# TianxiangZhao/EdgeDisentangle_SSL

Measured on NVIDIA B200. Metric: DISGAT fwd+bwd edges/s, higher is better.
Workload: dtype f32

## Files before the change

### edgedisentangle_ssl_b200/_lib.py

```python
import ctypes
import os
from ctypes import POINTER, Structure, c_char_p, c_double, c_float, c_int, c_int32, c_int64, c_uint64, c_void_p

_PKG = os.path.dirname(os.path.abspath(__file__))
LIB_PATH = os.environ.get("EDIS_LIB") or os.path.join(_PKG, "libedis.so")


class EdisError(RuntimeError):
    pass


class LayerDesc(Structure):
    _fields_ = [("att", c_int32), ("C", c_int32), ("D", c_int32), ("Dv", c_int32),
                ("training", c_int32), ("p", c_float), ("seed", c_uint64), ("flags", c_int32),
                ("reserved", c_int32)]


ERR_STALE = -5
FLAG_PLAIN_MEAN = 1
FLAG_NO_GX = 2
FLAG_PHASE_DST, FLAG_PHASE_SRC, FLAG_PHASE_GX = 4, 8, 16


def _load():
    if not os.path.exists(LIB_PATH):
        raise ImportError(
            "libedis.so not found at %s: build it with `python -m edgedisentangle_ssl_b200.build` "
            "(nvcc, sm_100a).  This package has no CPU / PyTorch fallback." % LIB_PATH)
    return ctypes.CDLL(LIB_PATH)


lib = _load()

_i64p = POINTER(c_int64)
_i32p = POINTER(c_int32)
_f32p = POINTER(c_float)
_f64p = POINTER(c_double)
_descp = POINTER(LayerDesc)
_P = c_void_p

_BWD_ARGS = [c_void_p, _descp, _P, c_int64, _P, c_int64, _P, _P, c_int64, _P, _P, _P, _P, _P, _P, _P,
             _P, c_int64, _P, c_int64, _P, _P, c_int64, _P, _P, _P, c_int64, _P]

SIGNATURES = {
    "edis_last_error": (c_char_p, []),
    "edis_version": (c_char_p, []),
    "edis_build_adjacency_host": (c_int64, [c_int64, c_int64, _i64p, _i64p, _f64p, _i64p, _i64p, _f32p]),
    "edis_graph_create": (c_int, [c_int64, c_int64, _i64p, _i64p, c_int, c_int, POINTER(c_void_p)]),
    "edis_graph_create_rect": (c_int, [c_int64, c_int64, c_int64, _i64p, _i64p, c_int, c_int, POINTER(c_void_p)]),
    "edis_graph_destroy": (None, [c_void_p]),
    "edis_graph_info": (c_int, [c_void_p, _i64p]),
    "edis_graph_input_entries": (c_int64, [c_void_p]),
    "edis_graph_export": (c_int, [c_void_p, _i64p, _i32p, _i64p, _i64p, _i32p, _i32p]),
    "edis_graph_workspace_bytes": (c_int64, [c_void_p, c_int64]),
    "edis_edge_list_key": (c_uint64, [c_int64, c_int64, c_int64, _i64p, _i64p, c_int]),
    "edis_graph_save": (c_int, [c_void_p, c_char_p, c_uint64]),
    "edis_graph_load": (c_int, [c_char_p, c_uint64, c_int, c_int, c_int, POINTER(c_void_p)]),
    "edis_disga_fwd": (c_int, [c_void_p, _descp, _P, c_int64, _P, c_int64, _P, _P, c_int64, _P,
                               _P, _P, _P, _P, _P, _P, c_int64, _P]),
    "edis_disga_rec_bytes": (c_int64, [c_void_p, _descp]),
    "edis_disga_sign_bytes": (c_int64, [c_void_p, _descp]),
    "edis_disga_bwd": (c_int, _BWD_ARGS),
    "edis_disga_bwd_dst": (c_int, _BWD_ARGS),
    "edis_disga_bwd_src": (c_int, _BWD_ARGS),
    "edis_disga_sage_fwd": (c_int, [c_void_p, _descp, _P, c_int64, _P, c_int64, _P, _P, c_int64,
                                    _P, _P, _P, _P, _P, c_int64, _P]),
    "edis_disga_sage_bwd": (c_int, [c_void_p, _descp, _P, c_int64, _P, c_int64, _P, _P, c_int64,
                                    _P, _P, _P, _P, _P, _P, _P, c_int64, _P, c_int64, _P, _P, _P, _P, _P,
                                    c_int64, _P]),
    "edis_disga_sage_fused_gx": (c_int, [_descp]),
    "edis_pair_score_fwd": (c_int, [_descp, c_int64, c_int64, _P, _P, c_int32, c_int32, _P, c_int64,
                                    _P, c_int64, _P, _P, _P, _P]),
    "edis_pair_score_bwd": (c_int, [_descp, c_int64, c_int64, _P, _P, c_int32, c_int32, _P, c_int64,
                                    _P, c_int64, _P, _P, _P, _P, _P, _P, _P, _P]),
    "edis_pair_sign_bytes": (c_int64, [_descp, c_int64, c_int32, c_int32]),
    "edis_ssl_wmse_fwd": (c_int, [c_int64, c_int32, _P, _P, c_int64, c_int64, _P, _P, c_int64, _P]),
    "edis_ssl_wmse_bwd": (c_int, [c_int64, c_int32, _P, _P, c_int64, c_int64, _P, _P, _P]),
    "edis_nll_const_label_fwd": (c_int, [c_int64, c_int32, _P, c_int32, _P, _P, c_int64, _P]),
    "edis_nll_const_label_bwd": (c_int, [c_int64, c_int32, _P, c_int32, _P, _P, _P]),
    "edis_sp_softmax_fwd": (c_int, [c_int64, c_int64, _P, _P, _P, _P, _P, _P]),
    "edis_sp_softmax_bwd": (c_int, [c_int64, c_int64, _P, _P, _P, _P, _P, _P]),
    "edis_sp_matmul_fwd": (c_int, [c_int64, c_int64, c_int64, _P, _P, _P, _P, _P, _P]),
    "edis_sp_matmul_bwd": (c_int, [c_int64, c_int64, c_int64, _P, _P, _P, _P, _P, _P, _P, _P]),
    "edis_merge_pairs_host": (c_int64, [c_int64, _i64p, c_int64, _i64p, c_int64, _i64p, _i64p, _f32p]),
    "edis_rand_hits_host": (c_int64, [c_void_p, c_int64, c_int64, ctypes.c_uint32, _i64p, c_int64]),
}

for _name, (_res, _args) in SIGNATURES.items():
    _fn = getattr(lib, _name)
    _fn.restype = _res
    _fn.argtypes = _args


def last_error():
    return lib.edis_last_error().decode("utf-8", "replace")


def check(status, what):
    if status is not None and status < 0:
        raise EdisError("%s failed (%d): %s" % (what, status, last_error()))
    return status


def np_ptr(arr, ctype):
    return arr.ctypes.data_as(POINTER(ctype))


def version():
    return lib.edis_version().decode()
```

### edgedisentangle_ssl_b200/functional.py

```python
import ctypes

import torch

from . import _lib
from ._lib import LayerDesc, check, lib


def _stream():
    return ctypes.c_void_p(torch.cuda.current_stream().cuda_stream)


def _ptr(t):
    return ctypes.c_void_p(t.data_ptr()) if t is not None else None


def _off(t, col):
    return ctypes.c_void_p(t.data_ptr() + 4 * int(col))


def _rows(t, what):
    if t.dtype != torch.float32 or not t.is_cuda:
        raise _lib.EdisError("%s must be a float32 CUDA tensor (got %s on %s)" % (what, t.dtype, t.device))
    if t.dim() != 2 or t.stride(1) != 1:
        t = t.contiguous()
    return t, t.stride(0)


class KernelTimer:

    def __init__(self):
        self.enabled = False
        self.records = {}
        self.launches = 0

    def reset(self):
        self.records = {}
        self.launches = 0

    def durations_ms(self):
        return {k: [a.elapsed_time(b) for a, b, _ in v] for k, v in self.records.items()}

    def bytes(self):
        return {k: [m for _, _, m in v] for k, v in self.records.items()}


TIMER = KernelTimer()


def kernel_bytes(kind, n, nc, e, att, C, D, Fin=None, sage=False):
    CD = C * D
    score = 4 * C if att == 1 else 4 * CD
    agg_ref = 4 * Fin if sage else 4 * CD
    agg_own = 4 * CD if Fin is None else 4 * Fin
    wout = CD if Fin is None else C * Fin
    sign = CD // 8 if att == 3 else 0
    if kind == "fwd":
        alg = e * (score + agg_ref + 4 * C + 4) + 8 * CD * n
        moved = e * (score + agg_own + 4 * C + sign + 4) + n * (score + 4 * wout * (1 if Fin else 2) + 8 * C)
    elif kind == "bwd_dst":
        alg = e * (score + agg_ref + 4 * C + 4) + 8 * CD * n
        moved = (e * ((score if att == 2 else 0) + agg_own + 4 * C + 8 * C + sign + 4)
                 + n * (12 * wout + 2 * score + 8 * C))
    elif kind == "bwd_src":
        alg = e * (score + agg_ref) + 4 * CD * n
        moved = (e * ((score if att == 2 else 0) + 4 * wout + 8 * C + sign + 8)
                 + nc * (score + (4 * CD if Fin is None else 4 * Fin)))
    elif kind == "bwd_src_score":
        alg = e * score + 4 * CD * n
        moved = e * ((score if att == 2 else 0) + 8 * C + sign + 8) + nc * score
    else:
        alg = e * agg_ref
        moved = e * (4 * wout + 4 * C + 8) + nc * 4 * Fin
    return {"alg": int(alg), "moved": int(moved)}


class _timed:
    def __init__(self, name, graph, launches, nbytes=None):
        self.name, self.launches, self.nbytes = name, launches, nbytes

    def __enter__(self):
        if TIMER.enabled:
            self.start = torch.cuda.Event(enable_timing=True)
            self.end = torch.cuda.Event(enable_timing=True)
            self.start.record(torch.cuda.current_stream())
        return self

    def __exit__(self, *exc):
        if TIMER.enabled:
            self.end.record(torch.cuda.current_stream())
            TIMER.records.setdefault(self.name, []).append((self.start, self.end, self.nbytes))
            TIMER.launches += self.launches
        return False


def phase(name):
    return _timed("phase:" + name, None, 0, None)


def _desc(att, C, D, training=False, p=0.0, seed=0):
    return LayerDesc(att=att, C=C, D=D, Dv=D, training=1 if (training and p > 0) else 0, p=float(p),
                     seed=int(seed) & 0xFFFFFFFFFFFFFFFF)


def _edge_rec(graph, d, device):
    nbytes = check(lib.edis_disga_rec_bytes(graph.handle, ctypes.byref(d)), "edis_disga_rec_bytes")
    return torch.empty(int(nbytes), dtype=torch.uint8, device=device)


def _sign_rec(graph, d, device, wanted):
    if d.att != 3 or not wanted:
        return None
    nbytes = check(lib.edis_disga_sign_bytes(graph.handle, ctypes.byref(d)), "edis_disga_sign_bytes")
    return torch.empty(int(nbytes), dtype=torch.uint8, device=device)


def _workspace(graph, width, like):
    nbytes = graph.workspace_bytes(width)
    return torch.empty(nbytes, dtype=torch.uint8, device=like.device), nbytes


def disga_forward_raw(graph, d, P, ldp, Q, ldq, V, ldv, a, bias, device, want_sign):
    C, D = d.C, d.D
    CD = C * D
    n, e = graph.n, graph.e
    out = torch.empty(n, CD, dtype=torch.float32, device=device)
    hpre = torch.empty_like(out)
    edge_e = torch.empty(e, C, dtype=torch.float32, device=device)
    stats = torch.empty(n, 2 * C, dtype=torch.float32, device=device)
    ws, nbytes = _workspace(graph, CD + 2 * C, out)
    esign = _sign_rec(graph, d, device, want_sign)
    with _timed("disga_fwd", graph, 1 + (1 if graph.info["dst_slots"] else 0),
                kernel_bytes("fwd", n, graph.n_cols, e, d.att, C, D)):
        check(lib.edis_disga_fwd(graph.handle, ctypes.byref(d), P, ldp, Q, ldq, _ptr(a), V, ldv, _ptr(bias),
                                 _ptr(out), _ptr(hpre), _ptr(edge_e), _ptr(stats), _ptr(esign), _ptr(ws), nbytes,
                                 _stream()), "edis_disga_fwd")
    return out, hpre, edge_e, stats, esign


def disga_backward_raw(graph, d, P, ldp, Q, ldq, V, ldv, a, bias, hpre, edge_e, stats, esign, g_out, g_edge_e,
                       gP, ldgp, gQ, ldgq, ga, gV, ldgv, device):
    C, D, att = d.C, d.D, d.att
    CD = C * D
    n, e, nc = graph.n, graph.e, graph.n_cols
    edge_rec = _edge_rec(graph, d, device)
    gh = torch.empty(n, CD, dtype=torch.float32, device=device)
    ws, nbytes = _workspace(graph, 2 * CD + 2 * C, gh)
    args = (graph.handle, ctypes.byref(d), P, ldp, Q, ldq, _ptr(a), V, ldv, _ptr(bias),
            _ptr(hpre), _ptr(edge_e), _ptr(stats), _ptr(esign), _ptr(g_out), _ptr(g_edge_e), gP, ldgp, gQ, ldgq,
            _ptr(ga), gV, ldgv, _ptr(edge_rec), _ptr(gh), _ptr(ws), nbytes, _stream())
    with _timed("disga_bwd_dst", graph, 1 + (1 if graph.info["dst_slots"] else 0),
                kernel_bytes("bwd_dst", n, nc, e, att, C, D)):
        check(lib.edis_disga_bwd_dst(*args), "edis_disga_bwd_dst")
    with _timed("disga_bwd_src", graph, 1 + (2 if graph.info["src_slots"] else 0),
                kernel_bytes("bwd_src", n, nc, e, att, C, D)):
        check(lib.edis_disga_bwd_src(*args), "edis_disga_bwd_src")
    return gh


class DisGAFused(torch.autograd.Function):

    @staticmethod
    def forward(ctx, graph, att, C, D, proj, off_p, off_q, off_v, sdst, ssrc, a, bias, training, p, seed):
        proj, ld = _rows(proj, "proj")
        if att == 1:
            sdst, ssrc = sdst.contiguous(), ssrc.contiguous()
            P, Q, ldp, ldq = _ptr(sdst), _ptr(ssrc), C, C
        else:
            P, Q, ldp, ldq = _off(proj, off_p), _off(proj, off_q), ld, ld
        a = a.contiguous() if a is not None else None
        bias = bias.contiguous() if bias is not None else None
        if proj.shape[0] != graph.n_cols:
            raise _lib.EdisError("projection has %d rows, graph has %d source nodes" % (proj.shape[0], graph.n_cols))
        d = _desc(att, C, D, training, p, seed)
        out, hpre, edge_e, stats, esign = disga_forward_raw(graph, d, P, ldp, Q, ldq, _off(proj, off_v), ld, a, bias,
                                                            proj.device, any(ctx.needs_input_grad))
        ctx.graph, ctx.d, ctx.offs = graph, d, (off_p, off_q, off_v)
        ctx.has_a, ctx.has_bias = a is not None, bias is not None
        ctx.save_for_backward(proj, sdst, ssrc, a, bias, hpre, edge_e, stats, esign)
        ctx.set_materialize_grads(False)
        return out, edge_e

    @staticmethod
    def backward(ctx, g_out, g_edge_e):
        proj, sdst, ssrc, a, bias, hpre, edge_e, stats, esign = ctx.saved_tensors
        graph, d = ctx.graph, ctx.d
        C, D, att = d.C, d.D, d.att
        CD = C * D
        n, e, nc = graph.n, graph.e, graph.n_cols
        rect = nc > n
        off_p, off_q, off_v = ctx.offs
        ld, W, dev = proj.stride(0), proj.shape[1], proj.device
        if g_out is None:
            g_out = torch.zeros(n, CD, dtype=torch.float32, device=dev)
        g_out = g_out.contiguous()
        if g_edge_e is not None:
            g_edge_e = g_edge_e.contiguous()
        g_sd = g_ss = gq_sep = None
        if att == 1:
            g_proj = torch.zeros(nc, W, dtype=torch.float32, device=dev)
            g_sd = (torch.zeros if rect else torch.empty)(nc, C, dtype=torch.float32, device=dev)
            g_ss = torch.empty(nc, C, dtype=torch.float32, device=dev)
            P, Q, ldp, ldq = _ptr(sdst), _ptr(ssrc), C, C
            gP, gQ, ldgp, ldgq = _ptr(g_sd), _ptr(g_ss), C, C
        else:
            covered = CD * (3 if att == 3 else 2)
            g_proj = (torch.empty if W == covered and not rect else torch.zeros)(nc, W, dtype=torch.float32,
                                                                                 device=dev)
            P, Q, ldp, ldq = _off(proj, off_p), _off(proj, off_q), ld, ld
            gP, ldgp = _off(g_proj, off_p), W
            if off_q == off_p:
                gq_sep = torch.empty(nc, CD, dtype=torch.float32, device=dev)
                gQ, ldgq = _ptr(gq_sep), CD
            else:
                gQ, ldgq = _off(g_proj, off_q), W
        ga = torch.zeros(C, D, dtype=torch.float32, device=dev) if att == 3 else None
        gh = disga_backward_raw(graph, d, P, ldp, Q, ldq, _off(proj, off_v), ld, a, bias, hpre, edge_e, stats, esign,
                                g_out, g_edge_e, gP, ldgp, gQ, ldgq, ga, _off(g_proj, off_v), W, dev)
        if gq_sep is not None:
            g_proj[:, off_p:off_p + CD] += gq_sep
        gbias = gh.sum(0) if ctx.has_bias else None
        return (None, None, None, None, g_proj, None, None, None, g_sd, g_ss,
                ga if ctx.has_a else None, gbias, None, None, None)


def sage_forward_raw(graph, d, P, ldp, Q, ldq, X, a, want_sign):
    n, e, Fin, C = graph.n, graph.e, X.shape[1], d.C
    if X.shape[0] != graph.n_cols:
        raise _lib.EdisError("X has %d rows, graph has %d source nodes" % (X.shape[0], graph.n_cols))
    agg = torch.empty(n, C * Fin, dtype=torch.float32, device=X.device)
    edge_e = torch.empty(e, C, dtype=torch.float32, device=X.device)
    stats = torch.empty(n, 2 * C, dtype=torch.float32, device=X.device)
    ws, nbytes = _workspace(graph, C * Fin + 2 * C, X)
    esign = _sign_rec(graph, d, X.device, want_sign)
    plain = bool(d.flags & _lib.FLAG_PLAIN_MEAN)
    with _timed("disga_sage_fwd", graph, 1 + (1 if graph.info["dst_slots"] else 0),
                kernel_bytes("fwd", n, graph.n_cols, e, d.att, C, d.D, Fin, sage=not plain)):
        check(lib.edis_disga_sage_fwd(graph.handle, ctypes.byref(d), P, ldp, Q, ldq, _ptr(a), _ptr(X), X.stride(0),
                                      _ptr(agg), _ptr(edge_e), _ptr(stats), _ptr(esign), _ptr(ws), nbytes,
                                      _stream()),
              "edis_disga_sage_fwd")
    return agg, edge_e, stats, esign


def sage_backward_raw(graph, d, P, ldp, Q, ldq, X, a, agg, edge_e, stats, esign, g_agg, g_edge_e, gP, ldgp, gQ, ldgq,
                      ga, need_gx):
    C, D, att, Fin = d.C, d.D, d.att, d.Dv
    CD = C * D
    n, e, nc = graph.n, graph.e, graph.n_cols
    dev = X.device
    gX = torch.empty(nc, Fin, dtype=torch.float32, device=dev) if need_gx else None
    edge_rec = _edge_rec(graph, d, dev)
    gh = torch.empty(n, C * Fin, dtype=torch.float32, device=dev)
    ws, nbytes = _workspace(graph, 2 * CD + 2 * C + Fin, X)
    base = d.flags
    plain = bool(base & _lib.FLAG_PLAIN_MEAN)
    fused_gx = bool(lib.edis_disga_sage_fused_gx(ctypes.byref(d)))
    kb = lambda kind: kernel_bytes(kind, n, nc, e, att, C, D, Fin, sage=not plain)
    phases = [("disga_sage_bwd_dst", _lib.FLAG_PHASE_DST, 1 + (1 if graph.info["dst_slots"] else 0), kb("bwd_dst")),
              ("disga_sage_bwd_src", _lib.FLAG_PHASE_SRC, 1 + (1 if graph.info["src_slots"] else 0),
               kb("bwd_src" if (fused_gx and need_gx) else "bwd_src_score"))]
    if need_gx and not fused_gx:
        phases.append(("disga_sage_bwd_gx", _lib.FLAG_PHASE_GX, 1 + (1 if graph.info["src_slots"] else 0),
                       kb("bwd_gx")))
    for name, bit, nl, nb in phases:
        d.flags = base | bit
        with _timed(name, graph, nl, nb):
            check(lib.edis_disga_sage_bwd(graph.handle, ctypes.byref(d), P, ldp, Q, ldq, _ptr(a), _ptr(X),
                                          X.stride(0), _ptr(agg), _ptr(edge_e), _ptr(stats), _ptr(esign), _ptr(g_agg),
                                          _ptr(g_edge_e), gP, ldgp, gQ, ldgq, _ptr(ga), _ptr(gX),
                                          _ptr(edge_rec), _ptr(gh), _ptr(ws), nbytes, _stream()),
                  "edis_disga_sage_bwd")
    d.flags = base
    return gX


class SageFused(torch.autograd.Function):

    @staticmethod
    def forward(ctx, graph, att, C, D, proj, off_p, off_q, sdst, ssrc, a, X, training, p, seed, plain):
        X, ldx = _rows(X, "X")
        if att == 1:
            sdst, ssrc = sdst.contiguous(), ssrc.contiguous()
            P, Q, ldp, ldq = _ptr(sdst), _ptr(ssrc), C, C
        else:
            proj, ld = _rows(proj, "proj")
            P, Q, ldp, ldq = _off(proj, off_p), _off(proj, off_q), ld, ld
        a = a.contiguous() if a is not None else None
        d = _desc(att, C, D, training, p, seed)
        d.Dv = X.shape[1]
        d.flags = (_lib.FLAG_PLAIN_MEAN if plain else 0) | (0 if ctx.needs_input_grad[10] else _lib.FLAG_NO_GX)
        agg, edge_e, stats, esign = sage_forward_raw(graph, d, P, ldp, Q, ldq, X, a, any(ctx.needs_input_grad))
        ctx.graph, ctx.d, ctx.offs, ctx.plain = graph, d, (off_p, off_q), bool(plain)
        ctx.has_a = a is not None
        ctx.save_for_backward(proj, sdst, ssrc, a, X, agg, edge_e, stats, esign)
        ctx.set_materialize_grads(False)
        return agg, edge_e

    @staticmethod
    def backward(ctx, g_agg, g_edge_e):
        proj, sdst, ssrc, a, X, agg, edge_e, stats, esign = ctx.saved_tensors
        graph, d = ctx.graph, ctx.d
        C, D, att = d.C, d.D, d.att
        CD = C * D
        n, nc = graph.n, graph.n_cols
        rect = nc > n
        off_p, off_q = ctx.offs
        dev = X.device
        if g_agg is None:
            g_agg = torch.zeros_like(agg)
        g_agg = g_agg.contiguous()
        if g_edge_e is not None:
            g_edge_e = g_edge_e.contiguous()
        g_proj = g_sd = g_ss = gq_sep = None
        if att == 1:
            g_sd = (torch.zeros if rect else torch.empty)(nc, C, dtype=torch.float32, device=dev)
            g_ss = torch.empty(nc, C, dtype=torch.float32, device=dev)
            P, Q, ldp, ldq = _ptr(sdst), _ptr(ssrc), C, C
            gP, gQ, ldgp, ldgq = _ptr(g_sd), _ptr(g_ss), C, C
        else:
            ld, W = proj.stride(0), proj.shape[1]
            covered = CD * (2 if att == 3 else 1)
            g_proj = (torch.empty if W == covered and not rect else torch.zeros)(nc, W, dtype=torch.float32,
                                                                                 device=dev)
            P, Q, ldp, ldq = _off(proj, off_p), _off(proj, off_q), ld, ld
            gP, ldgp = _off(g_proj, off_p), W
            if off_q == off_p:
                gq_sep = torch.empty(nc, CD, dtype=torch.float32, device=dev)
                gQ, ldgq = _ptr(gq_sep), CD
            else:
                gQ, ldgq = _off(g_proj, off_q), W
        need_gx = not (d.flags & _lib.FLAG_NO_GX)
        ga = torch.zeros(C, D, dtype=torch.float32, device=dev) if att == 3 else None
        gX = sage_backward_raw(graph, d, P, ldp, Q, ldq, X, a, agg, edge_e, stats, esign, g_agg, g_edge_e, gP, ldgp,
                               gQ, ldgq, ga, need_gx)
        if gq_sep is not None:
            g_proj[:, off_p:off_p + CD] += gq_sep
        return (None, None, None, None, g_proj, None, None, g_sd, g_ss, ga if ctx.has_a else None, gX,
                None, None, None, None)


PROJ3X_MIN_ROWS = 65536


def use_proj3x(n_rows):
    import os
    mode = os.environ.get("EDIS_PROJ3X", "auto")
    return mode == "1" or (mode != "0" and n_rows >= PROJ3X_MIN_ROWS)


def _tf32_hi(t):
    return ((t.view(torch.int32) + 0x1000) & -0x2000).view(torch.float32)


def _xt_g(x, g, chunks=256):
    n = x.shape[0]
    if n < chunks * 1024:
        return x.t() @ g
    m = (n // chunks) * chunks
    out = torch.bmm(x[:m].view(chunks, m // chunks, -1).transpose(1, 2), g[:m].view(chunks, m // chunks, -1)).sum(0)
    if m < n:
        out += x[m:].t() @ g[m:]
    return out


class Proj3xTF32(torch.autograd.Function):

    @staticmethod
    def forward(ctx, x, w):
        xh, wh = _tf32_hi(x), _tf32_hi(w)
        xc = torch.cat([xh, xh, x - xh], 1)
        wc = torch.cat([wh, w - wh, wh], 0)
        prev = torch.backends.cuda.matmul.allow_tf32
        torch.backends.cuda.matmul.allow_tf32 = True
        try:
            out = xc @ wc
        finally:
            torch.backends.cuda.matmul.allow_tf32 = prev
        ctx.save_for_backward(x, w)
        return out

    @staticmethod
    def backward(ctx, g):
        x, w = ctx.saved_tensors
        gx = g @ w.t() if ctx.needs_input_grad[0] else None
        gw = _xt_g(x, g) if ctx.needs_input_grad[1] else None
        return gx, gw


def _mm_3xtf32(x, w):
    xh, wh = _tf32_hi(x), _tf32_hi(w)
    xc = torch.cat([xh, xh, x - xh], 1)
    wc = torch.cat([wh, w - wh, wh], 0)
    prev = torch.backends.cuda.matmul.allow_tf32
    torch.backends.cuda.matmul.allow_tf32 = True
    try:
        return xc @ wc
    finally:
        torch.backends.cuda.matmul.allow_tf32 = prev


class NodeLinear(torch.autograd.Function):

    @staticmethod
    def forward(ctx, x, weight, bias):
        ctx.save_for_backward(x, weight)
        ctx.has_bias = bias is not None
        return torch.nn.functional.linear(x, weight, bias)

    @staticmethod
    def backward(ctx, g):
        x, weight = ctx.saved_tensors
        g = g.contiguous()
        gx = gw = gb = None
        if ctx.needs_input_grad[0]:
            gx = _mm_3xtf32(g, weight) if weight.shape[0] <= 128 else g @ weight
        if ctx.needs_input_grad[1]:
            gw = _xt_g(g, x)
        if ctx.has_bias and ctx.needs_input_grad[2]:
            gb = g.sum(0)
        return gx, gw, gb


def node_linear(lin, x):
    if x.is_cuda and x.dim() == 2 and x.shape[0] >= 262144 and x.dtype == torch.float32:
        return NodeLinear.apply(x, lin.weight, lin.bias)
    return lin(x)


class ChannelLinear(torch.autograd.Function):

    @staticmethod
    def forward(ctx, agg, W):
        C, Fin, D = W.shape
        out = torch.empty(agg.shape[0], C * D, dtype=agg.dtype, device=agg.device)
        for c in range(C):
            torch.mm(agg[:, c * Fin:(c + 1) * Fin], W[c], out=out[:, c * D:(c + 1) * D])
        ctx.save_for_backward(agg, W)
        return out

    @staticmethod
    def backward(ctx, g):
        agg, W = ctx.saved_tensors
        C, Fin, D = W.shape
        g = g.contiguous()
        g_agg = torch.empty_like(agg) if ctx.needs_input_grad[0] else None
        g_w = torch.empty_like(W) if ctx.needs_input_grad[1] else None
        for c in range(C):
            gc = g[:, c * D:(c + 1) * D]
            if g_agg is not None:
                torch.mm(gc, W[c].t(), out=g_agg[:, c * Fin:(c + 1) * Fin])
            if g_w is not None:
                torch.mm(agg[:, c * Fin:(c + 1) * Fin].t(), gc, out=g_w[c])
        return g_agg, g_w


class PairList:

    def __init__(self, pairs):
        self.pi, self.pj = pairs[0].contiguous(), pairs[1].contiguous()
        self._perm = None

    @staticmethod
    def wrap(p):
        return p if isinstance(p, PairList) else PairList(p)

    def col_perm(self):
        if self._perm is None:
            self._perm = torch.sort(self.pj.to(torch.int32))[1].to(torch.int32)
        return self._perm


class PairScore(torch.autograd.Function):

    @staticmethod
    def forward(ctx, att, C, D, pi, pj, c_lo, c_hi, P, Q, a, plist=None):
        P, ldp = _rows(P, "P")
        Q, ldq = _rows(Q, "Q")
        a = a.contiguous() if a is not None else None
        pi = pi.contiguous()
        pj = pj.contiguous()
        if pi.dtype != torch.int64 or pj.dtype != torch.int64 or not pi.is_cuda:
            raise _lib.EdisError("pair indices must be int64 CUDA tensors")
        m, n = pi.numel(), P.shape[0]
        out = torch.empty(m, c_hi - c_lo, dtype=torch.float32, device=P.device)
        d = _desc(att, C, D)
        psign = None
        if att == 3 and any(ctx.needs_input_grad) and 0 < m < 2 ** 31 and ldp % 4 == 0 and ldq % 4 == 0 \
                and P.data_ptr() % 16 == 0 and Q.data_ptr() % 16 == 0:
            nb = check(lib.edis_pair_sign_bytes(ctypes.byref(d), m, c_lo, c_hi), "edis_pair_sign_bytes")
            psign = torch.empty(int(nb), dtype=torch.uint8, device=P.device)
        with _timed("pair_fwd", None, 1):
            check(lib.edis_pair_score_fwd(ctypes.byref(d), n, m, _ptr(pi), _ptr(pj), c_lo, c_hi, _ptr(P), ldp,
                                          _ptr(Q), ldq, _ptr(a), _ptr(out), _ptr(psign), _stream()),
                  "edis_pair_score_fwd")
        ctx.d, ctx.rng, ctx.lds = d, (c_lo, c_hi), (ldp, ldq)
        ctx.has_a = a is not None
        ctx.plist = plist if plist is not None else (PairList(torch.stack([pi, pj])) if psign is not None else None)
        ctx.save_for_backward(pi, pj, P, Q, a, psign)
        return out

    @staticmethod
    def backward(ctx, g_out):
        pi, pj, P, Q, a, psign = ctx.saved_tensors
        d = ctx.d
        c_lo, c_hi = ctx.rng
        ldp, ldq = ctx.lds
        n, m = P.shape[0], pi.numel()
        wdt = d.C if d.att == 1 else d.C * d.D
        gP = torch.zeros(n, wdt, dtype=torch.float32, device=P.device)
        gQ = torch.zeros(Q.shape[0], wdt, dtype=torch.float32, device=P.device)
        ga = torch.zeros(d.C, d.D, dtype=torch.float32, device=P.device) if d.att == 3 else None
        g_out = g_out.contiguous()
        perm = ctx.plist.col_perm() if psign is not None else None
        with _timed("pair_bwd", None, 2 if psign is not None else 1):
            check(lib.edis_pair_score_bwd(ctypes.byref(d), n, m, _ptr(pi), _ptr(pj), c_lo, c_hi, _ptr(P), ldp,
                                          _ptr(Q), ldq, _ptr(a), _ptr(g_out), _ptr(psign), _ptr(perm), _ptr(gP),
                                          _ptr(gQ), _ptr(ga), _stream()), "edis_pair_score_bwd")
        return (None, None, None, None, None, None, None, gP, gQ, ga if ctx.has_a else None, None)


class SslWmse(torch.autograd.Function):

    @staticmethod
    def forward(ctx, scores, target, n_pos, m_total=None):
        scores = scores.contiguous()
        target = target.contiguous()
        m, cs = scores.shape
        m_total = m if m_total is None else int(m_total)
        ctx.n_pos, ctx.m_total = int(n_pos), m_total
        if m == 0:
            ctx.save_for_backward(scores, target)
            return scores.new_zeros(())
        loss = torch.empty(1, dtype=torch.float32, device=scores.device)
        ws = torch.empty(8, dtype=torch.uint8, device=scores.device)
        check(lib.edis_ssl_wmse_fwd(m, cs, _ptr(scores), _ptr(target), int(n_pos), m_total, _ptr(loss), _ptr(ws), 8,
                                    _stream()), "edis_ssl_wmse_fwd")
        ctx.n_pos, ctx.m_total = int(n_pos), m_total
        ctx.save_for_backward(scores, target)
        return loss.reshape(())

    @staticmethod
    def backward(ctx, g_loss):
        scores, target = ctx.saved_tensors
        m, cs = scores.shape
        if m == 0:
            return torch.zeros_like(scores), None, None, None
        g_scores = torch.empty_like(scores)
        g_loss = g_loss.reshape(1).contiguous().float()
        check(lib.edis_ssl_wmse_bwd(m, cs, _ptr(scores), _ptr(target), ctx.n_pos, ctx.m_total, _ptr(g_loss),
                                    _ptr(g_scores), _stream()), "edis_ssl_wmse_bwd")
        return g_scores, None, None, None


class NllConstLabel(torch.autograd.Function):

    @staticmethod
    def forward(ctx, logits, label):
        logits = logits.contiguous()
        n, k = logits.shape
        loss = torch.empty(1, dtype=torch.float32, device=logits.device)
        ws = torch.empty(8, dtype=torch.uint8, device=logits.device)
        check(lib.edis_nll_const_label_fwd(n, k, _ptr(logits), int(label), _ptr(loss), _ptr(ws), 8, _stream()),
              "edis_nll_const_label_fwd")
        ctx.label = int(label)
        ctx.save_for_backward(logits)
        return loss.reshape(())

    @staticmethod
    def backward(ctx, g_loss):
        (logits,) = ctx.saved_tensors
        n, k = logits.shape
        g_logits = torch.empty_like(logits)
        g_loss = g_loss.reshape(1).contiguous().float()
        check(lib.edis_nll_const_label_bwd(n, k, _ptr(logits), ctx.label, _ptr(g_loss), _ptr(g_logits),
                                           _stream()), "edis_nll_const_label_bwd")
        return g_logits, None


class SpSoftmax(torch.autograd.Function):

    @staticmethod
    def forward(ctx, row, values, n):
        shape = values.shape
        v = values.reshape(-1).contiguous()
        row = row.contiguous()
        out = torch.empty_like(v)
        denom = torch.empty(n, dtype=torch.float32, device=v.device)
        vmax = torch.empty(1, dtype=torch.float32, device=v.device)
        check(lib.edis_sp_softmax_fwd(n, v.numel(), _ptr(row), _ptr(v), _ptr(out), _ptr(denom), _ptr(vmax),
                                      _stream()), "edis_sp_softmax_fwd")
        ctx.n, ctx.shape = n, shape
        ctx.save_for_backward(row, out)
        return out.reshape(shape)

    @staticmethod
    def backward(ctx, g):
        row, out = ctx.saved_tensors
        g = g.reshape(-1).contiguous()
        gv = torch.empty_like(out)
        rowdot = torch.empty(ctx.n, dtype=torch.float32, device=out.device)
        check(lib.edis_sp_softmax_bwd(ctx.n, out.numel(), _ptr(row), _ptr(out), _ptr(g), _ptr(gv), _ptr(rowdot),
                                      _stream()), "edis_sp_softmax_bwd")
        return None, gv.reshape(ctx.shape), None


class SpMatmul(torch.autograd.Function):

    @staticmethod
    def forward(ctx, row, col, values, mat):
        v = values.reshape(-1).contiguous()
        mat = mat.contiguous()
        row, col = row.contiguous(), col.contiguous()
        n, f = mat.shape
        out = torch.empty_like(mat)
        check(lib.edis_sp_matmul_fwd(n, v.numel(), f, _ptr(row), _ptr(col), _ptr(v), _ptr(mat), _ptr(out),
                                     _stream()), "edis_sp_matmul_fwd")
        ctx.vshape = values.shape
        ctx.save_for_backward(row, col, v, mat)
        return out

    @staticmethod
    def backward(ctx, g):
        row, col, v, mat = ctx.saved_tensors
        n, f = mat.shape
        g = g.contiguous()
        gv = torch.empty_like(v)
        gm = torch.empty_like(mat)
        check(lib.edis_sp_matmul_bwd(n, v.numel(), f, _ptr(row), _ptr(col), _ptr(v), _ptr(mat), _ptr(g),
                                     _ptr(gv), _ptr(gm), _stream()), "edis_sp_matmul_bwd")
        return None, None, gv.reshape(ctx.vshape), gm
```

### include/edis.h

```cpp
#ifndef EDIS_H_
#define EDIS_H_

#include <stdint.h>

#ifdef __cplusplus
extern "C" {
#endif

#define EDIS_OK 0
#define EDIS_ERR_ARG (-1)
#define EDIS_ERR_CUDA (-2)
#define EDIS_ERR_UNSUPPORTED (-3)
#define EDIS_ERR_WORKSPACE (-4)
#define EDIS_ERR_STALE (-5)

const char* edis_last_error(void);
const char* edis_version(void);

int64_t edis_build_adjacency_host(int64_t n, int64_t m, const int64_t* rows, const int64_t* cols,
                                  const double* vals, int64_t* out_row, int64_t* out_col,
                                  float* out_val);

typedef struct edis_graph edis_graph;
int edis_graph_create(int64_t n, int64_t e, const int64_t* row, const int64_t* col, int max_chunk,
                      int device, edis_graph** out);
int edis_graph_create_rect(int64_t n_rows, int64_t n_cols, int64_t e, const int64_t* row,
                           const int64_t* col, int max_chunk, int device, edis_graph** out);
void edis_graph_destroy(edis_graph* g);

int edis_graph_info(const edis_graph* g, int64_t info[10]);
int64_t edis_graph_input_entries(const edis_graph* g);
int edis_graph_export(const edis_graph* g, int64_t* rowptr, int32_t* col, int64_t* perm,
                      int64_t* cscptr, int32_t* cscrow, int32_t* csceid);
int64_t edis_graph_workspace_bytes(const edis_graph* g, int64_t width);

uint64_t edis_edge_list_key(int64_t n, int64_t n_cols, int64_t e_in, const int64_t* row,
                            const int64_t* col, int max_chunk);
int edis_graph_save(const edis_graph* g, const char* path, uint64_t key);
int edis_graph_load(const char* path, uint64_t key, int max_chunk, int device, int verify,
                    edis_graph** out);

typedef struct {
  int32_t att;
  int32_t C;
  int32_t D;
  int32_t Dv;
  int32_t training;
  float p;
  uint64_t seed;
  int32_t flags;
  int32_t reserved;
} edis_layer_desc;
#define EDIS_FLAG_PLAIN_MEAN 1
#define EDIS_FLAG_NO_GX 2
#define EDIS_FLAG_PHASE_DST 4
#define EDIS_FLAG_PHASE_SRC 8
#define EDIS_FLAG_PHASE_GX 16
#define EDIS_FLAG_PHASE_MASK 28

int edis_disga_fwd(const edis_graph* g, const edis_layer_desc* d,
                   const float* P, int64_t ldp, const float* Q, int64_t ldq, const float* a,
                   const float* V, int64_t ldv, const float* bias,
                   float* out, float* hpre, float* edge_e, float* stats, uint8_t* esign,
                   void* workspace, int64_t workspace_bytes, void* stream);
int64_t edis_disga_sign_bytes(const edis_graph* g, const edis_layer_desc* d);

int edis_disga_bwd(const edis_graph* g, const edis_layer_desc* d,
                   const float* P, int64_t ldp, const float* Q, int64_t ldq, const float* a,
                   const float* V, int64_t ldv, const float* bias,
                   const float* hpre, const float* edge_e, const float* stats, const uint8_t* esign,
                   const float* g_out, const float* g_edge_e,
                   float* gP, int64_t ldgp, float* gQ, int64_t ldgq, float* ga, float* gV, int64_t ldgv,
                   float* edge_rec, float* gh,
                   void* workspace, int64_t workspace_bytes, void* stream);
int64_t edis_disga_rec_bytes(const edis_graph* g, const edis_layer_desc* d);
int edis_disga_bwd_dst(const edis_graph* g, const edis_layer_desc* d,
                       const float* P, int64_t ldp, const float* Q, int64_t ldq, const float* a,
                       const float* V, int64_t ldv, const float* bias,
                       const float* hpre, const float* edge_e, const float* stats, const uint8_t* esign,
                       const float* g_out, const float* g_edge_e,
                       float* gP, int64_t ldgp, float* gQ, int64_t ldgq, float* ga, float* gV, int64_t ldgv,
                       float* edge_rec, float* gh,
                       void* workspace, int64_t workspace_bytes, void* stream);
int edis_disga_bwd_src(const edis_graph* g, const edis_layer_desc* d,
                       const float* P, int64_t ldp, const float* Q, int64_t ldq, const float* a,
                       const float* V, int64_t ldv, const float* bias,
                       const float* hpre, const float* edge_e, const float* stats, const uint8_t* esign,
                       const float* g_out, const float* g_edge_e,
                       float* gP, int64_t ldgp, float* gQ, int64_t ldgq, float* ga, float* gV, int64_t ldgv,
                       float* edge_rec, float* gh,
                       void* workspace, int64_t workspace_bytes, void* stream);

int edis_disga_sage_fwd(const edis_graph* g, const edis_layer_desc* d,
                        const float* P, int64_t ldp, const float* Q, int64_t ldq, const float* a,
                        const float* X, int64_t ldx,
                        float* neigh, float* edge_e, float* stats, uint8_t* esign,
                        void* workspace, int64_t workspace_bytes, void* stream);
int edis_disga_sage_bwd(const edis_graph* g, const edis_layer_desc* d,
                        const float* P, int64_t ldp, const float* Q, int64_t ldq, const float* a,
                        const float* X, int64_t ldx,
                        const float* neigh, const float* edge_e, const float* stats, const uint8_t* esign,
                        const float* g_neigh, const float* g_edge_e,
                        float* gP, int64_t ldgp, float* gQ, int64_t ldgq, float* ga, float* gX,
                        float* edge_rec, float* gh,
                        void* workspace, int64_t workspace_bytes, void* stream);

int edis_disga_sage_fused_gx(const edis_layer_desc* d);

int edis_pair_score_fwd(const edis_layer_desc* d, int64_t n, int64_t m, const int64_t* pi,
                        const int64_t* pj, int32_t c_lo, int32_t c_hi,
                        const float* P, int64_t ldp, const float* Q, int64_t ldq, const float* a,
                        float* out, uint8_t* psign, void* stream);
int edis_pair_score_bwd(const edis_layer_desc* d, int64_t n, int64_t m, const int64_t* pi,
                        const int64_t* pj, int32_t c_lo, int32_t c_hi,
                        const float* P, int64_t ldp, const float* Q, int64_t ldq, const float* a,
                        const float* g_out, const uint8_t* psign, const int32_t* col_perm,
                        float* gP, float* gQ, float* ga, void* stream);
int64_t edis_pair_sign_bytes(const edis_layer_desc* d, int64_t m, int32_t c_lo, int32_t c_hi);

int edis_ssl_wmse_fwd(int64_t m, int32_t cs, const float* scores, const float* target,
                      int64_t n_pos, int64_t m_total, float* loss, void* workspace,
                      int64_t workspace_bytes, void* stream);
int edis_ssl_wmse_bwd(int64_t m, int32_t cs, const float* scores, const float* target,
                      int64_t n_pos, int64_t m_total, const float* g_loss, float* g_scores,
                      void* stream);

int edis_nll_const_label_fwd(int64_t n, int32_t k, const float* logits, int32_t label,
                             float* loss, void* workspace, int64_t workspace_bytes, void* stream);
int edis_nll_const_label_bwd(int64_t n, int32_t k, const float* logits, int32_t label,
                             const float* g_loss, float* g_logits, void* stream);

int edis_sp_softmax_fwd(int64_t n, int64_t e, const int64_t* row, const float* values,
                        float* out, float* denom, float* vmax, void* stream);
int edis_sp_softmax_bwd(int64_t n, int64_t e, const int64_t* row, const float* out,
                        const float* g_out, float* g_values, float* rowdot, void* stream);
int edis_sp_matmul_fwd(int64_t n, int64_t e, int64_t f, const int64_t* row, const int64_t* col,
                       const float* values, const float* mat, float* out, void* stream);
int edis_sp_matmul_bwd(int64_t n, int64_t e, int64_t f, const int64_t* row, const int64_t* col,
                       const float* values, const float* mat, const float* g_out,
                       float* g_values, float* g_mat, void* stream);

int64_t edis_merge_pairs_host(int64_t n_hit, const int64_t* hit_key, int64_t n_forced,
                              const int64_t* forced_key, int64_t n_pos, const int64_t* pos_key,
                              int64_t* out_key, float* out_label);

int64_t edis_rand_hits_host(uint8_t* state, int64_t state_bytes, int64_t n_draws, uint32_t thr24,
                            int64_t* out, int64_t cap);

#ifdef __cplusplus
}
#endif
#endif
```

Measured before the change: 267.5 million.

## Add tcgen05 split-K 3xTF32 kernel for tall-skinny X^T G weight gradients

Replaces the chunked bmm-plus-sum path for X^T·G weight gradients with a custom Blackwell kernel for large row counts. The kernel splits K into slabs, converts fp32 rows to TF32 hi/lo pairs in shared memory and issues three tcgen05 MMAs per step into double-buffered TMEM accumulators. Converter warps drain TMEM into register accumulators, and a second kernel reduces the slab partials in double. This aims to cut the memory and launch overhead of the bmm path while keeping near-fp32 accuracy, at the cost of a workspace allocation per call and a hand-built UMMA pipeline that must get its descriptors right.

```diff
diff --git a/edgedisentangle_ssl_b200/_lib.py b/edgedisentangle_ssl_b200/_lib.py
--- a/edgedisentangle_ssl_b200/_lib.py
+++ b/edgedisentangle_ssl_b200/_lib.py
@@ -82,6 +82,8 @@
     "edis_sp_softmax_bwd": (c_int, [c_int64, c_int64, _P, _P, _P, _P, _P, _P]),
     "edis_sp_matmul_fwd": (c_int, [c_int64, c_int64, c_int64, _P, _P, _P, _P, _P, _P]),
     "edis_sp_matmul_bwd": (c_int, [c_int64, c_int64, c_int64, _P, _P, _P, _P, _P, _P, _P, _P]),
+    "edis_xtg_3xtf32_workspace_bytes": (c_int64, [c_int64, c_int64, c_int64]),
+    "edis_xtg_3xtf32": (c_int, [c_int64, c_int64, c_int64, _P, c_int64, _P, c_int64, _P, _P, c_int64, _P]),
     "edis_merge_pairs_host": (c_int64, [c_int64, _i64p, c_int64, _i64p, c_int64, _i64p, _i64p, _f32p]),
     "edis_rand_hits_host": (c_int64, [c_void_p, c_int64, c_int64, ctypes.c_uint32, _i64p, c_int64]),
 }
diff --git a/edgedisentangle_ssl_b200/csrc/gemm.cu b/edgedisentangle_ssl_b200/csrc/gemm.cu
--- /dev/null
+++ b/edgedisentangle_ssl_b200/csrc/gemm.cu
@@ -0,0 +1,338 @@
+#include "edis_common.cuh"
+
+#include <algorithm>
+
+namespace edis {
+namespace {
+
+constexpr int kRows = 16;
+constexpr int kStages = 4;
+constexpr int kLoadAhead = 3;
+constexpr int kSubSteps = 8;
+constexpr int kMaxNarrow = 128;
+constexpr int kChunks = kMaxNarrow / 8 / 4;
+constexpr int kSlabs = 256;
+constexpr int kMaxChain = 8192;
+constexpr int kPrefetch = 8;
+constexpr int kConvThreads = 512;
+constexpr int kThreads = kConvThreads + 32;
+constexpr int kWide = 128;
+static_assert(kWide * (kRows / 4) == kConvThreads, "one wide task per converter thread");
+static_assert(kMaxNarrow * (kRows / 4) <= kConvThreads, "at most one narrow task per converter thread");
+
+struct XtgArgs {
+  const float* wide;
+  const float* narrow;
+  int64_t ld_wide, ld_narrow, k, chain;
+  int n_wide, n_narrow, n_umma, n_groups;
+  float* partial;
+};
+
+__device__ __forceinline__ void mbar_arrive(uint32_t bar) {
+  asm volatile("mbarrier.arrive.shared::cta.b64 _, [%0];" ::"r"(bar) : "memory");
+}
+__device__ __forceinline__ void fence_async_smem() { asm volatile("fence.proxy.async.shared::cta;" ::: "memory"); }
+__device__ __forceinline__ void tc_fence_before() { asm volatile("tcgen05.fence::before_thread_sync;" ::: "memory"); }
+__device__ __forceinline__ void tc_fence_after() { asm volatile("tcgen05.fence::after_thread_sync;" ::: "memory"); }
+__device__ __forceinline__ void tc_commit(uint32_t bar) {
+  asm volatile("tcgen05.commit.cta_group::1.mbarrier::arrive::one.shared::cluster.b64 [%0];" ::"r"(bar) : "memory");
+}
+__device__ __forceinline__ void umma_tf32(uint32_t d_tmem, uint64_t a_desc, uint64_t b_desc, uint32_t idesc,
+                                          uint32_t accumulate) {
+  asm volatile(
+      "{\n.reg .pred p;\n"
+      "setp.ne.b32 p, %4, 0;\n"
+      "tcgen05.mma.cta_group::1.kind::tf32 [%0], %1, %2, %3, p;\n"
+      "}\n" ::"r"(d_tmem), "l"(a_desc), "l"(b_desc), "r"(idesc), "r"(accumulate)
+      : "memory");
+}
+__device__ __forceinline__ void tmem_ld8(uint32_t taddr, float (&v)[8]) {
+  uint32_t r[8];
+  asm volatile("tcgen05.ld.sync.aligned.32x32b.x8.b32 {%0, %1, %2, %3, %4, %5, %6, %7}, [%8];"
+               : "=r"(r[0]), "=r"(r[1]), "=r"(r[2]), "=r"(r[3]), "=r"(r[4]), "=r"(r[5]), "=r"(r[6]), "=r"(r[7])
+               : "r"(taddr));
+  asm volatile("tcgen05.wait::ld.sync.aligned;" ::: "memory");
+#pragma unroll
+  for (int i = 0; i < 8; ++i) v[i] = __uint_as_float(r[i]);
+}
+
+__device__ __forceinline__ uint64_t smem_desc(uint32_t addr, uint32_t lbo, uint32_t sbo) {
+  return static_cast<uint64_t>((addr >> 4) & 0x3FFF) | static_cast<uint64_t>((lbo >> 4) & 0x3FFF) << 16 |
+         static_cast<uint64_t>((sbo >> 4) & 0x3FFF) << 32 | 1ull << 46;
+}
+__host__ __device__ constexpr uint32_t idesc_tf32(int n) {
+  return (1u << 4) | (2u << 7) | (2u << 10) | (static_cast<uint32_t>(n >> 3) << 17) | ((128u >> 4) << 24);
+}
+
+__device__ __forceinline__ float tf32_rn(float v) {
+  return __uint_as_float((__float_as_uint(v) + 0x1000u) & 0xFFFFE000u);
+}
+
+struct Tile {
+  uint32_t hi, lo, rows;
+};
+
+__device__ __forceinline__ void load_task(float (&v)[4], const float* base, int64_t ld, int64_t row, int64_t k_end,
+                                          bool col_ok) {
+#pragma unroll
+  for (int r = 0; r < 4; ++r)
+    v[r] = (col_ok && row + r < k_end) ? __ldg(base + (row + r) * ld) : 0.0f;
+}
+__device__ __forceinline__ void prefetch_task(const float* base, int64_t ld, int64_t row, int64_t k_end, bool col_ok) {
+#pragma unroll
+  for (int r = 0; r < 4; ++r)
+    if (col_ok && row + r < k_end) asm volatile("prefetch.global.L2 [%0];" ::"l"(base + (row + r) * ld));
+}
+__device__ __forceinline__ void store_task(const float (&v)[4], const Tile& t, uint32_t rg, uint32_t c) {
+  float h[4], l[4];
+#pragma unroll
+  for (int r = 0; r < 4; ++r) {
+    h[r] = tf32_rn(v[r]);
+    l[r] = tf32_rn(v[r] - h[r]);
+  }
+  const uint32_t off = rg * t.rows * 16 + c * 16;
+  asm volatile("st.shared.v4.f32 [%0], {%1, %2, %3, %4};" ::"r"(t.hi + off), "f"(h[0]), "f"(h[1]), "f"(h[2]), "f"(h[3])
+               : "memory");
+  asm volatile("st.shared.v4.f32 [%0], {%1, %2, %3, %4};" ::"r"(t.lo + off), "f"(l[0]), "f"(l[1]), "f"(l[2]), "f"(l[3])
+               : "memory");
+}
+
+__global__ void __launch_bounds__(kThreads, 1) k_xtg_3xtf32(XtgArgs A) {
+  extern __shared__ __align__(1024) unsigned char smem_raw[];
+  __shared__ uint64_t full_bar[kStages], empty_bar[kStages], acc_full[2], acc_empty[2];
+  __shared__ uint32_t tmem_base;
+
+  const int tid = threadIdx.x, warp = tid >> 5;
+  const int slab = blockIdx.x / A.n_groups, group = blockIdx.x % A.n_groups;
+  const int64_t k_beg = static_cast<int64_t>(slab) * A.chain;
+  const int64_t k_end = min(A.k, k_beg + A.chain);
+  const int n_steps = static_cast<int>((k_end - k_beg + kRows - 1) / kRows);
+  const int n_sub = (n_steps + kSubSteps - 1) / kSubSteps;
+  const int nu = A.n_umma;
+  const uint32_t wide_bytes = kWide * kRows * 4, narrow_bytes = nu * kRows * 4;
+  const uint32_t stage_bytes = 2 * (wide_bytes + narrow_bytes);
+  const uint32_t smem0 = smem_u32(smem_raw);
+  const uint32_t acc_cols = nu <= 32 ? 32 : nu <= 64 ? 64 : 128;
+
+  if (warp == kConvThreads / 32) {
+    if (tid % 32 == 0) {
+      for (int s = 0; s < kStages; ++s) {
+        mbar_init(smem_u32(&full_bar[s]), kConvThreads);
+        mbar_init(smem_u32(&empty_bar[s]), 1);
+      }
+      for (int b = 0; b < 2; ++b) {
+        mbar_init(smem_u32(&acc_full[b]), 1);
+        mbar_init(smem_u32(&acc_empty[b]), kConvThreads);
+      }
+      mbar_fence_init();
+    }
+    __syncwarp();
+    asm volatile("tcgen05.alloc.cta_group::1.sync.aligned.shared::cta.b32 [%0], %1;" ::"r"(smem_u32(&tmem_base)),
+                 "r"(2 * acc_cols)
+                 : "memory");
+    asm volatile("tcgen05.relinquish_alloc_permit.cta_group::1.sync.aligned;" ::: "memory");
+  }
+  tc_fence_before();
+  __syncthreads();
+  tc_fence_after();
+  const uint32_t tmem = tmem_base;
+
+  if (warp < kConvThreads / 32) {
+    const float* wbase = A.wide + static_cast<int64_t>(group) * kWide;
+    const int wcols = min(kWide, A.n_wide - group * kWide);
+    const int np = (A.n_narrow + 31) & ~31;
+    const int cw = tid % kWide, rgw = tid / kWide;
+    const int cn = tid % np, rgn = tid / np;
+    const bool wide_ok = cw < wcols, narrow_ok = tid < np * (kRows / 4) && cn < A.n_narrow;
+    const bool narrow_st = tid < np * (kRows / 4) && cn < nu;
+    auto load = [&](float (&v)[2][4], int step) {
+      const int64_t row0 = k_beg + static_cast<int64_t>(step) * kRows;
+      load_task(v[0], wbase + cw, A.ld_wide, row0 + 4 * rgw, k_end, wide_ok && step < n_steps);
+      load_task(v[1], A.narrow + cn, A.ld_narrow, row0 + 4 * rgn, k_end, narrow_ok && step < n_steps);
+    };
+    auto prefetch = [&](int step) {
+      const int64_t row0 = k_beg + static_cast<int64_t>(step) * kRows;
+      prefetch_task(wbase + cw, A.ld_wide, row0 + 4 * rgw, k_end, wide_ok && step < n_steps);
+      prefetch_task(A.narrow + cn, A.ld_narrow, row0 + 4 * rgn, k_end, narrow_ok && step < n_steps);
+    };
+    const int q = warp & 3, part = warp >> 2;
+    float acc[kChunks][8];
+#pragma unroll
+    for (int c = 0; c < kChunks; ++c)
+#pragma unroll
+      for (int e = 0; e < 8; ++e) acc[c][e] = 0.0f;
+    int drained = 0;
+    auto drain = [&]() {
+      const int b = drained & 1;
+      mbar_wait(smem_u32(&acc_full[b]), (drained >> 1) & 1);
+      tc_fence_after();
+#pragma unroll
+      for (int c = 0; c < kChunks; ++c) {
+        const int ch = part + 4 * c;
+        if (ch < nu / 8) {
+          float v[8];
+          tmem_ld8(tmem + (static_cast<uint32_t>(32 * q) << 16) + b * acc_cols + 8 * ch, v);
+#pragma unroll
+          for (int e = 0; e < 8; ++e) acc[c][e] += v[e];
+        }
+      }
+      tc_fence_before();
+      mbar_arrive(smem_u32(&acc_empty[b]));
+      ++drained;
+    };
+
+    float regs[kLoadAhead][2][4];
+    for (int p = 0; p < kPrefetch; ++p) prefetch(p);
+#pragma unroll
+    for (int d = 0; d < kLoadAhead; ++d) load(regs[d], d);
+    for (int i0 = 0; i0 < n_steps; i0 += kLoadAhead) {
+#pragma unroll
+      for (int d = 0; d < kLoadAhead; ++d) {
+        const int i = i0 + d;
+        if (i < n_steps) {
+          prefetch(i + kPrefetch);
+          const int s = i % kStages;
+          if (i >= kStages) mbar_wait(smem_u32(&empty_bar[s]), ((i / kStages) - 1) & 1);
+          const uint32_t st = smem0 + s * stage_bytes;
+          store_task(regs[d][0], Tile{st, st + wide_bytes, kWide}, rgw, cw);
+          if (narrow_st)
+            store_task(regs[d][1], Tile{st + 2 * wide_bytes, st + 2 * wide_bytes + narrow_bytes, static_cast<uint32_t>(nu)},
+                       rgn, cn);
+          fence_async_smem();
+          mbar_arrive(smem_u32(&full_bar[s]));
+          load(regs[d], i + kLoadAhead);
+          if ((i + 1) % kSubSteps == 0 && i + 1 >= 2 * kSubSteps) drain();
+        }
+      }
+    }
+    while (drained < n_sub) drain();
+
+    const int m = group * kWide + 32 * q + (tid & 31);
+    if (m < A.n_wide) {
+      float* prow = A.partial + (static_cast<int64_t>(slab) * A.n_wide + m) * A.n_narrow;
+#pragma unroll
+      for (int c = 0; c < kChunks; ++c) {
+        const int ch = part + 4 * c;
+#pragma unroll
+        for (int e = 0; e < 8; ++e)
+          if (ch < nu / 8 && 8 * ch + e < A.n_narrow) prow[8 * ch + e] = acc[c][e];
+      }
+    }
+  } else if (tid % 32 == 0) {
+    const uint32_t idesc = idesc_tf32(nu);
+    for (int i = 0; i < n_steps; ++i) {
+      const int s = i % kStages, j = i / kSubSteps, b = j & 1;
+      const uint32_t d_tmem = tmem + b * acc_cols;
+      if (i % kSubSteps == 0 && j >= 2) {
+        mbar_wait(smem_u32(&acc_empty[b]), ((j >> 1) - 1) & 1);
+        tc_fence_after();
+      }
+      mbar_wait(smem_u32(&full_bar[s]), (i / kStages) & 1);
+      tc_fence_after();
+      const uint32_t st = smem0 + s * stage_bytes;
+      const uint32_t wh = st, wl = st + wide_bytes, nh = st + 2 * wide_bytes, nl = nh + narrow_bytes;
+#pragma unroll
+      for (int ks = 0; ks < kRows / 8; ++ks) {
+        const uint32_t wo = ks * 2 * kWide * 16, no = ks * 2 * nu * 16;
+        const uint64_t dwh = smem_desc(wh + wo, kWide * 16, 128), dwl = smem_desc(wl + wo, kWide * 16, 128);
+        const uint64_t dnh = smem_desc(nh + no, nu * 16, 128), dnl = smem_desc(nl + no, nu * 16, 128);
+        umma_tf32(d_tmem, dwh, dnh, idesc, (i % kSubSteps) != 0 || ks != 0);
+        umma_tf32(d_tmem, dwh, dnl, idesc, 1);
+        umma_tf32(d_tmem, dwl, dnh, idesc, 1);
+      }
+      tc_commit(smem_u32(&empty_bar[s]));
+      if ((i + 1) % kSubSteps == 0 || i + 1 == n_steps) tc_commit(smem_u32(&acc_full[b]));
+    }
+  }
+
+  tc_fence_before();
+  __syncthreads();
+  if (warp == kConvThreads / 32) {
+    tc_fence_after();
+    asm volatile("tcgen05.dealloc.cta_group::1.sync.aligned.b32 %0, %1;" ::"r"(tmem), "r"(2 * acc_cols) : "memory");
+  }
+}
+
+__global__ void k_xtg_reduce(const float* __restrict__ partial, int n_slabs, int n_wide, int n_narrow, bool trans,
+                             float* __restrict__ c) {
+  const int64_t per = static_cast<int64_t>(n_wide) * n_narrow;
+  const int64_t e = static_cast<int64_t>(blockIdx.x) * blockDim.x + threadIdx.x;
+  if (e >= per) return;
+  double acc = 0.0;
+#pragma unroll 8
+  for (int s = 0; s < n_slabs; ++s) acc += partial[s * per + e];
+  const int64_t w = e / n_narrow, n = e % n_narrow;
+  c[trans ? n * n_wide + w : e] = static_cast<float>(acc);
+}
+
+int launch_xtg(const XtgArgs& A, int n_slabs, cudaStream_t stream) {
+  const size_t smem = static_cast<size_t>(kStages) * 2 * (kWide + A.n_umma) * kRows * 4;
+  EDIS_CUDA(cudaFuncSetAttribute(k_xtg_3xtf32, cudaFuncAttributeMaxDynamicSharedMemorySize, static_cast<int>(smem)));
+  k_xtg_3xtf32<<<n_slabs * A.n_groups, kThreads, smem, stream>>>(A);
+  EDIS_CUDA(cudaGetLastError());
+  return EDIS_OK;
+}
+
+int64_t xtg_chain(int64_t k) { return std::min<int64_t>(kMaxChain, ((k + kSlabs - 1) / kSlabs + kRows - 1) / kRows * kRows); }
+int64_t xtg_slabs(int64_t k) { return (k + xtg_chain(k) - 1) / xtg_chain(k); }
+
+int xtg_shape(const char* who, int64_t k, int64_t m, int64_t n) {
+  EDIS_CHECK_ARG(k > 0 && m > 0 && n > 0, "%s: bad sizes K=%lld M=%lld N=%lld", who, (long long)k, (long long)m,
+                 (long long)n);
+  if (std::min(m, n) > kMaxNarrow) {
+    set_error("%s: unsupported shape M=%lld N=%lld (the narrow side must be <= %d columns)", who, (long long)m,
+              (long long)n, kMaxNarrow);
+    return EDIS_ERR_UNSUPPORTED;
+  }
+  EDIS_CHECK_ARG(std::max(m, n) < (int64_t(1) << 24) && xtg_slabs(k) * ((std::max(m, n) + kWide - 1) / kWide) < (int64_t(1) << 31),
+                 "%s: sizes out of range", who);
+  return EDIS_OK;
+}
+
+}
+}
+
+using namespace edis;
+
+extern "C" int64_t edis_xtg_3xtf32_workspace_bytes(int64_t k, int64_t m, int64_t n) {
+  const int rc = xtg_shape("edis_xtg_3xtf32_workspace_bytes", k, m, n);
+  if (rc) return rc;
+  return xtg_slabs(k) * m * n * 4;
+}
+
+extern "C" int edis_xtg_3xtf32(int64_t k, int64_t m, int64_t n, const float* a, int64_t lda, const float* b,
+                               int64_t ldb, float* c, void* workspace, int64_t workspace_bytes, void* stream) {
+  const char* who = "edis_xtg_3xtf32";
+  const int rc = xtg_shape(who, k, m, n);
+  if (rc) return rc;
+  EDIS_CHECK_ARG(a && b && c && workspace, "%s: null pointer", who);
+  EDIS_CHECK_ARG(lda >= m && ldb >= n, "%s: row strides (%lld, %lld) below the widths (%lld, %lld)", who,
+                 (long long)lda, (long long)ldb, (long long)m, (long long)n);
+  const int64_t need = edis_xtg_3xtf32_workspace_bytes(k, m, n);
+  if (workspace_bytes < need) {
+    set_error("%s: workspace too small (%lld < %lld)", who, (long long)workspace_bytes, (long long)need);
+    return EDIS_ERR_WORKSPACE;
+  }
+  const bool trans = m <= n;
+  XtgArgs A = {};
+  A.wide = trans ? b : a;
+  A.narrow = trans ? a : b;
+  A.ld_wide = trans ? ldb : lda;
+  A.ld_narrow = trans ? lda : ldb;
+  A.k = k;
+  A.chain = xtg_chain(k);
+  A.n_wide = static_cast<int>(trans ? n : m);
+  A.n_narrow = static_cast<int>(trans ? m : n);
+  A.n_umma = (A.n_narrow + 15) & ~15;
+  A.n_groups = (A.n_wide + kWide - 1) / kWide;
+  A.partial = static_cast<float*>(workspace);
+  const int n_slabs = static_cast<int>(xtg_slabs(k));
+  cudaStream_t s = static_cast<cudaStream_t>(stream);
+  const int r = launch_xtg(A, n_slabs, s);
+  if (r) return r;
+  const int64_t per = static_cast<int64_t>(m) * n;
+  k_xtg_reduce<<<static_cast<unsigned>((per + 255) / 256), 256, 0, s>>>(A.partial, n_slabs, A.n_wide, A.n_narrow,
+                                                                         trans, c);
+  EDIS_CUDA(cudaGetLastError());
+  return EDIS_OK;
+}
diff --git a/edgedisentangle_ssl_b200/functional.py b/edgedisentangle_ssl_b200/functional.py
--- a/edgedisentangle_ssl_b200/functional.py
+++ b/edgedisentangle_ssl_b200/functional.py
@@ -352,15 +352,22 @@
     return ((t.view(torch.int32) + 0x1000) & -0x2000).view(torch.float32)
 
 
-def _xt_g(x, g, chunks=256):
+XTG_MIN_ROWS = 262144
+
+
+def _xt_g(x, g):
     n = x.shape[0]
-    if n < chunks * 1024:
-        return x.t() @ g
-    m = (n // chunks) * chunks
-    out = torch.bmm(x[:m].view(chunks, m // chunks, -1).transpose(1, 2), g[:m].view(chunks, m // chunks, -1)).sum(0)
-    if m < n:
-        out += x[m:].t() @ g[m:]
-    return out
+    if (n >= XTG_MIN_ROWS and x.is_cuda and x.device == g.device and x.dtype == g.dtype == torch.float32
+            and x.dim() == g.dim() == 2 and g.shape[0] == n and x.stride(1) == 1 and g.stride(1) == 1):
+        m, w = x.shape[1], g.shape[1]
+        nbytes = lib.edis_xtg_3xtf32_workspace_bytes(n, m, w)
+        if nbytes >= 0:
+            ws = torch.empty(nbytes, dtype=torch.uint8, device=x.device)
+            out = torch.empty(m, w, dtype=torch.float32, device=x.device)
+            check(lib.edis_xtg_3xtf32(n, m, w, _ptr(x), x.stride(0), _ptr(g), g.stride(0), _ptr(out), _ptr(ws),
+                                      nbytes, _stream()), "edis_xtg_3xtf32")
+            return out
+    return x.t() @ g
 
 
 class Proj3xTF32(torch.autograd.Function):
diff --git a/include/edis.h b/include/edis.h
--- a/include/edis.h
+++ b/include/edis.h
@@ -140,6 +140,10 @@
                        const float* values, const float* mat, const float* g_out,
                        float* g_values, float* g_mat, void* stream);
 
+int64_t edis_xtg_3xtf32_workspace_bytes(int64_t k, int64_t m, int64_t n);
+int edis_xtg_3xtf32(int64_t k, int64_t m, int64_t n, const float* a, int64_t lda, const float* b,
+                    int64_t ldb, float* c, void* workspace, int64_t workspace_bytes, void* stream);
+
 int64_t edis_merge_pairs_host(int64_t n_hit, const int64_t* hit_key, int64_t n_forced,
                               const int64_t* forced_key, int64_t n_pos, const int64_t* pos_key,
                               int64_t* out_key, float* out_label);
diff --git a/profiles/xtg_bench.py b/profiles/xtg_bench.py
--- /dev/null
+++ b/profiles/xtg_bench.py
@@ -0,0 +1,84 @@
+import argparse
+import os
+import subprocess
+import sys
+
+import torch
+
+sys.path.insert(0, os.path.dirname(os.path.dirname(os.path.abspath(__file__))))
+from edgedisentangle_ssl_b200 import functional as Fn
+
+SHAPES = [("layer1 x[K,100]^T gProj[K,1536]", 100, 1536),
+          ("layer2 x[K,64]^T gProj[K,1536]", 64, 1536),
+          ("fuser1 g[K,64]^T h[K,512]", 64, 512),
+          ("fuser2 g[K,64]^T h[K,512]", 64, 512)]
+
+
+def slab_bmm(x, g, chunks=256):
+    n = x.shape[0]
+    m = (n // chunks) * chunks
+    out = torch.bmm(x[:m].view(chunks, m // chunks, -1).transpose(1, 2), g[:m].view(chunks, m // chunks, -1)).sum(0)
+    if m < n:
+        out += x[m:].t() @ g[m:]
+    return out
+
+
+def time_ms(fn, reps):
+    ev = [torch.cuda.Event(enable_timing=True) for _ in range(2)]
+    ev[0].record()
+    for _ in range(reps):
+        fn()
+    ev[1].record()
+    ev[1].synchronize()
+    return ev[0].elapsed_time(ev[1]) / reps
+
+
+def errors(got, ref, terms):
+    err = (got.double() - ref).abs()
+    return (err / terms.clamp_min(1e-300)).max().item(), (err.max() / ref.abs().max()).item()
+
+
+def main():
+    ap = argparse.ArgumentParser()
+    ap.add_argument("--k", type=int, default=2_400_000)
+    ap.add_argument("--reps", type=int, default=10, help="launches per timed window")
+    ap.add_argument("--rounds", type=int, default=5, help="alternating old / new windows per shape")
+    a = ap.parse_args()
+    if not torch.cuda.is_available():
+        raise SystemExit("xtg_bench needs a CUDA device")
+    q = subprocess.run(["nvidia-smi", "--query-gpu=name,power.limit,clocks.max.sm", "--format=csv,noheader"],
+                       capture_output=True, text=True).stdout.strip().splitlines()
+    print("device: %s | nvidia-smi name, power.limit, clocks.max.sm: %s" % (torch.cuda.get_device_name(0),
+                                                                          q[0] if q else "n/a"))
+    print("K = %d, %d launches per window, %d alternating windows per path" % (a.k, a.reps, a.rounds))
+    print("%-34s %10s %10s %8s %11s %11s %11s %11s %9s" % ("product", "old ms", "new ms", "speedup", "old e/terms",
+                                                          "new e/terms", "old e/ref", "new e/ref", "new GB/s"))
+    tot_old = tot_new = 0.0
+    gen = torch.Generator(device="cuda").manual_seed(0)
+    for name, m, n in SHAPES:
+        x = torch.randn(a.k, m, device="cuda", generator=gen)
+        g = torch.randn(a.k, n, device="cuda", generator=gen)
+        new = Fn._xt_g(x, g)
+        old = slab_bmm(x, g)
+        ref = x.double().t() @ g.double()
+        terms = x.double().abs().t() @ g.double().abs()
+        e_old, e_new = errors(old, ref, terms), errors(new, ref, terms)
+        del ref, terms
+        t_old, t_new = [], []
+        for _ in range(a.rounds):
+            t_old.append(time_ms(lambda: slab_bmm(x, g), a.reps))
+            t_new.append(time_ms(lambda: Fn._xt_g(x, g), a.reps))
+        mo, mn = sorted(t_old)[len(t_old) // 2], sorted(t_new)[len(t_new) // 2]
+        tot_old += mo
+        tot_new += mn
+        gbs = (x.numel() + g.numel()) * 4 / (mn * 1e-3) / 1e9
+        print("%-34s %10.3f %10.3f %7.2fx %11.2e %11.2e %11.2e %11.2e %9.0f" % (name, mo, mn, mo / mn, e_old[0], e_new[0],
+                                                                             e_old[1], e_new[1], gbs))
+        print("    spread (min..max ms): old %.3f..%.3f  new %.3f..%.3f" % (min(t_old), max(t_old), min(t_new), max(t_new)))
+        del x, g
+        torch.cuda.empty_cache()
+    print("total of the four products: old %.2f ms, new %.2f ms (%.2fx)" % (tot_old, tot_new, tot_old / tot_new))
+
+
+if __name__ == "__main__":
+    main()
```

Result: slower. 254.7 million (median of 6 runs) (-4.8%).
